# OpenMatchmaking/microservice-matchmaking

Measured on AMD Instinct MI355X. Metric: matched players/sec over 1M-player pool, higher is better.
Workload: dtype int32

## Files before the change

microservice_matchmaking_amd/csrc/mm_engine.hip:

```cpp
#include <hip/hip_runtime.h>

#include <stdint.h>
#include <stdio.h>
#include <stdlib.h>
#include <string.h>
#include <time.h>

#include <dlfcn.h>

#include <algorithm>
#include <mutex>
#include <cmath>
#include <new>
#include <vector>

#include "../../include/mm_engine.h"
#include "../../include/mm_wait.h"
#include <mm_gfx950.h>


#define MM_NO_SLOT 0xFFFFFFFFu
#define MM_ST_FREE 0
#define MM_ST_LIVE 1
#define MM_ST_CANCELLED 2
// ... 841 lines not shown
    hipStream_t stream;
    hipEvent_t ev[4];
    hipEvent_t ev_nx[2];
    bool ev_nx_set;
    hipEvent_t ev_grp[MM_MAX_GROUPS];
    int last_hip;
    int32_t* d_q_rating;
    uint32_t* d_q_cons;
    uint32_t* d_q_slot;
    ChainDev* d_chains;
    uint8_t* d_state;
    uint32_t* d_released;
    uint32_t* d_counters;
    uint32_t* d_wave_hist;
    size_t wave_hist_rows;
    int32_t* d_in_rating;
    uint32_t* d_in_cons;
    uint8_t* d_in_group;
    uint32_t* d_in_slot;
    uint32_t* d_in_sel;
    size_t in_cap;
    uint32_t* d_in_stamp;
    size_t in_stamp_cap;
    uint32_t* d_out_slots;
    float* d_out_score;
    uint32_t* d_out_pass;
    uint32_t out_slot_stride, out_rec_stride;
    PairChain* d_pchains;
    uint32_t* d_pk_key[2];
    uint32_t* d_pk_oidx[2];
    uint16_t* d_pk_nx16[2];
    uint32_t* d_pk_bits[2];
    uint32_t* d_pk_scratch;
    uint16_t* d_pk_wpre;
    uint16_t* d_pk_g16;
    uint32_t* d_pk_rec1;
    uint16_t* d_pk_exa[2];
    uint32_t* d_pk_bitsp[2];
    uint32_t* d_pk_headp[2];
    bool kp_rounds_off;
    uint32_t pair_pcool;
    uint32_t pair_pstops;
    unsigned long long* d_pk_pbar;
    uint32_t round_ctr;
    uint32_t* d_pk_tilectl;
    uint32_t* d_pack;
    uint4* d_pk_grec;
    uint32_t pk_gstride;
    PairChain* h_pchains;
    uint32_t* h_look_seq;
    uint32_t look_seq;
    uint32_t ps_hand[4][MM_MAX_GROUPS];
    mm_path_stats ps;
    mm_tuning tn;
    uint32_t pk_bits_stride, pk_max_tiles, pk_stride;
    unsigned long long live_upper;
    TeamChain* d_tchains;
    TeamChain* h_tchains;
    uint32_t* d_tk_chunk;
    uint32_t* d_tk_fv2;
    uint32_t* d_tk_fpos;
    uint16_t* d_tk_memb;
    uint32_t* d_tk_bitsB;
    uint32_t* d_tk_chunkB;
    uint32_t* d_tk_fdone;
    uint32_t team_seq;
    uint32_t* d_tk_sqi;
// ... 445 lines not shown
    MMTRY(dev_alloc(e, e->d_q_rating, e->n_chains * cap * sizeof(int32_t)));
    MMTRY(dev_alloc(e, e->d_q_cons, e->n_chains * cap * sizeof(uint32_t)));
    MMTRY(dev_alloc(e, e->d_q_slot, e->n_chains * cap * sizeof(uint32_t)));
    MMTRY(dev_alloc(e, e->d_chains, e->n_chains * sizeof(ChainDev)));
    MMTRY(dev_alloc(e, e->d_state, cap));
    MMTRY(dev_alloc(e, e->d_released, (cap + 64) * sizeof(uint32_t)));
    MMTRY(dev_alloc(e, e->d_pack, (size_t)MM_PACK_MAX * (MM_MAX_LOBBY + 2u) * sizeof(uint32_t)));
    MMTRY(dev_alloc(e, e->d_counters, 2 * sizeof(uint32_t)));
    e->out_slot_stride = (uint32_t)(cap + 64);
    e->out_rec_stride = (uint32_t)(cap / 2 + 16);
    MMTRY(dev_alloc(e, e->d_out_slots, (size_t)cfg->n_groups * e->out_slot_stride * sizeof(uint32_t)));
    MMTRY(dev_alloc(e, e->d_out_score, (size_t)cfg->n_groups * e->out_rec_stride * sizeof(float)));
    MMTRY(dev_alloc(e, e->d_out_pass, (size_t)cfg->n_groups * e->out_rec_stride * sizeof(uint32_t)));
    {
        e->pk_stride = (uint32_t)((cap + 63) & ~(size_t)63);
        const size_t gc = (size_t)cfg->n_groups * e->pk_stride;
        e->pk_bits_stride = (uint32_t)(cap / 32 + 4);
        MMTRY(dev_alloc(e, e->d_pchains, cfg->n_groups * sizeof(PairChain)));
        e->pk_max_tiles = (uint32_t)(cap / (PK_TMAX / 4u) + 2);
        for (int b = 0; b < 2; ++b) {
            MMTRY(dev_alloc(e, e->d_pk_key[b], (gc + 64) * sizeof(uint32_t)));
            MMTRY(dev_alloc(e, e->d_pk_oidx[b], gc * sizeof(uint32_t)));
            MMTRY(dev_alloc(e, e->d_pk_nx16[b], (gc + 64) * sizeof(uint16_t)));
            MMTRY(dev_alloc(e, e->d_pk_bits[b], (size_t)cfg->n_groups * e->pk_bits_stride * sizeof(uint32_t)));
        }
        MMTRY(dev_alloc(e, e->d_pk_scratch, gc * sizeof(uint32_t)));
        MMTRY(dev_alloc(e, e->d_pk_g16, (gc + 64) * sizeof(uint16_t)));
        MMTRY(dev_alloc(e, e->d_pk_rec1, gc * sizeof(uint32_t)));
        for (int b = 0; b < 2; ++b) {
            MMTRY(dev_alloc(e, e->d_pk_exa[b], (gc + 64) * sizeof(uint16_t)));
            MMTRY(dev_alloc(e, e->d_pk_bitsp[b], (size_t)cfg->n_groups * e->pk_bits_stride * sizeof(uint32_t)));
            MMTRY(dev_alloc(e, e->d_pk_headp[b], (size_t)cfg->n_groups * e->pk_max_tiles * sizeof(uint32_t)));
        }
        MMTRY(dev_alloc(e, e->d_pk_wpre, (size_t)cfg->n_groups * e->pk_bits_stride * sizeof(uint16_t)));
        MMTRY(dev_alloc(e, e->d_pk_tilectl, (size_t)TC_N * cfg->n_groups * e->pk_max_tiles * sizeof(uint32_t)));
        MMTRY(dev_alloc(e, e->d_pk_pbar, (size_t)MM_MAX_GROUPS * 2u * sizeof(unsigned long long) + 64u));
        e->pk_gstride = (uint32_t)(2u * (e->pk_stride / PK_GS) + 4u * PK_TMAX);
        MMTRY(dev_alloc(e, e->d_pk_grec, (size_t)cfg->n_groups * e->pk_gstride * sizeof(uint4)));
        HIPCHK(e, hipMemsetAsync(e->d_pk_grec, 0xFF, (size_t)cfg->n_groups * e->pk_gstride * sizeof(uint4), e->stream));
        MMTRY(pin_alloc(e, e->h_pchains, cfg->n_groups * sizeof(PairChain)));
        MMTRY(pin_alloc(e, e->h_rslots, (cap + (size_t)3 * MM_MAX_LOBBY * cfg->n_groups + 64) * sizeof(uint32_t)));
        MMTRY(pin_alloc(e, e->h_rscore, (cap / 2 + (size_t)3 * MM_MAX_LOBBY * cfg->n_groups + 64) * sizeof(float)));
        MMTRY(pin_alloc(e, e->h_rpass, (cap / 2 + (size_t)3 * MM_MAX_LOBBY * cfg->n_groups + 64) * sizeof(uint32_t)));
        HIPCHK(e, hipMemsetAsync(e->d_pchains, 0, cfg->n_groups * sizeof(PairChain), e->stream));
        e->tk_chunk_stride = (uint32_t)(e->pk_stride / TT_CH + 2);
        MMTRY(dev_alloc(e, e->d_tchains, cfg->n_groups * sizeof(TeamChain)));
        MMTRY(dev_alloc(e, e->d_tk_chunk, (size_t)cfg->n_groups * MM_MAX_ROLES * e->tk_chunk_stride * sizeof(uint32_t)));
        MMTRY(dev_alloc(e, e->d_tk_fv2, gc * sizeof(uint32_t)));
        e->tk_memb = 0;
        for (uint32_t k = 0; k < cfg->n_modes; ++k) {
            const uint32_t L = cfg->modes[k].teams * cfg->modes[k].team_size;
            if (L > 2u && L - 1u > e->tk_memb) e->tk_memb = L - 1u;
        }
        if (e->tk_memb) {
            MMTRY(dev_alloc(e, e->d_tk_fpos, gc * sizeof(uint32_t)));
            MMTRY(dev_alloc(e, e->d_tk_memb, gc * e->tk_memb * sizeof(uint16_t)));
            MMTRY(dev_alloc(e, e->d_tk_bitsB, (size_t)cfg->n_groups * e->pk_bits_stride * sizeof(uint32_t)));
            MMTRY(dev_alloc(e, e->d_tk_chunkB, (size_t)cfg->n_groups * MM_MAX_ROLES * e->tk_chunk_stride * sizeof(uint32_t)));
            MMTRY(dev_alloc(e, e->d_tk_sqi, gc * sizeof(uint32_t)));
            MMTRY(dev_alloc(e, e->d_tk_fdone, (size_t)cfg->n_groups * e->tk_chunk_stride * sizeof(uint32_t)));
            HIPCHK(e, hipMemsetAsync(e->d_tk_fdone, 0, (size_t)cfg->n_groups * e->tk_chunk_stride * sizeof(uint32_t), e->stream));
        }
        MMTRY(pin_alloc(e, e->h_tchains, cfg->n_groups * sizeof(TeamChain)));
        HIPCHK(e, hipMemsetAsync(e->d_tchains, 0, cfg->n_groups * sizeof(TeamChain), e->stream));
    }
    MMTRY(pin_alloc(e, e->h_chains, e->n_chains * sizeof(ChainDev)));
    MMTRY(pin_alloc(e, e->h_look_seq, 64));
// ... 485 lines not shown
    P.out_rec_stride = e->out_rec_stride;
    P.chains = e->d_chains;
    P.q_rating = e->d_q_rating;
    P.q_cons = e->d_q_cons;
    P.q_slot = e->d_q_slot;
    P.state = e->d_state;
    P.released = e->d_released;
    P.n_released = e->d_counters;
    P.out_slots = e->d_out_slots;
    P.out_score = e->d_out_score;
    P.out_pass = e->d_out_pass;
}

static int pair_walk(mm_engine* e, uint32_t mode, const ModeDev& M, bool purge)
{
    const mm_config& cfg = e->cfg;
    const uint32_t G = cfg.n_groups;
    PairParams P;
    walk_params_common(P, e, mode, purge);
    P.tune = e->tn.pair_tune;
    P.pinject = e->tn.pair_pinject;
    P.ptimeout0 = e->tn.pair_ptimeout_us * 100u;
    P.ptimeout1 = P.ptimeout0 * 40u;
    P.window = M.window > 0xFFFFFu ? 0xFFFFFu : M.window;
    P.eqmask = M.eqmask;
    P.bits_stride = e->pk_bits_stride;
    P.pstride = e->pk_stride;
    P.pchains = e->d_pchains;
    for (int b = 0; b < 2; ++b) {
        P.key[b] = e->d_pk_key[b]; P.oidx[b] = e->d_pk_oidx[b];
        P.nx16[b] = e->d_pk_nx16[b]; P.bits[b] = e->d_pk_bits[b];
    }
    P.scratch = e->d_pk_scratch;
    P.wpre = e->d_pk_wpre;
    P.g16 = e->d_pk_g16;
    P.rec2[0] = e->d_pk_scratch;
    P.rec2[1] = e->d_pk_rec1;
    for (int b = 0; b < 2; ++b) { P.exa[b] = e->d_pk_exa[b]; P.bitsp[b] = e->d_pk_bitsp[b]; P.headp[b] = e->d_pk_headp[b]; }
    P.tilectl = e->d_pk_tilectl;
    P.max_tiles = e->pk_max_tiles;
    P.grec = e->d_pk_grec;
    P.gstride = e->pk_gstride;
    P.grp = 0;
    P.pbar = e->d_pk_pbar;
    P.pxmask = (uint32_t*)(e->d_pk_pbar + MM_MAX_GROUPS);
    P.pyield = (uint32_t*)(e->d_pk_pbar + MM_MAX_GROUPS) + MM_MAX_GROUPS;
    const unsigned long long bound64 = e->live_upper < cfg.capacity ? e->live_upper : cfg.capacity;
    const uint32_t bound = (uint32_t)bound64;
    if (e->tn.pair_tune & 0x10000u) HIPCHK(e, hipMemsetAsync(e->d_pk_grec, 0, (size_t)G * e->pk_gstride * sizeof(uint4), e->stream));
    hipLaunchKernelGGL(kp_init, dim3(G), dim3(1024), 0, e->stream, P, cfg.capacity);
    hipLaunchKernelGGL(kp_pack, dim3((bound + 32u + 1023u) / 1024u, G), dim3(1024), 0, e->stream, P);
    {
        uint32_t seg = 256u, stage = NXI_STAGE;
        while (seg < NXI_SEG && (unsigned long long)bound > 8192ull * seg) seg <<= 1;
        if (e->tn.pair_nxseg) seg = e->tn.pair_nxseg;
        if (e->tn.pair_nxstage) stage = e->tn.pair_nxstage;
        if (stage < seg + 64u) stage = seg + 64u;
        if (stage > NXI_STAGE) stage = NXI_STAGE;
        const bool timing = (cfg.flags & MM_CFG_TIMING) != 0;
        if (timing) HIPCHK(e, hipEventRecord(e->ev_nx[0], e->stream));
        hipLaunchKernelGGL(kp_nx_init, dim3((bound + seg - 1u) / seg + 1u, G), dim3(NXI_THREADS), 0, e->stream, P, seg, stage);
        if (timing) { HIPCHK(e, hipEventRecord(e->ev_nx[1], e->stream)); e->ev_nx_set = true; }
    }
    HIPCHK(e, hipGetLastError());
    uint32_t tail_no[MM_MAX_GROUPS];
    bool tail_send = false;
    memset(e->ps_hand, 0, sizeof(e->ps_hand));
    if (bound >= PL_MAX) {
        uint32_t tiles = (bound + PK_T - 1u) / PK_T + 1u;
        if (tiles > e->pk_max_tiles) tiles = e->pk_max_tiles;
        bool after_persist = false;
        uint32_t last_tp = 0;
        uint32_t idle_looks = 0;
        unsigned long long last_progress = ~0ull;
        for (uint32_t guard = 0;; ++guard) {
            if (idle_looks > 64u) return MM_ERR_INTERNAL;
            MMTRY(look_launch(e, e->d_pchains, e->h_pchains, G * sizeof(PairChain)));
            MMTRY(look_wait(e));
            ++e->ps.host_looks;
            if (e->tn.debug && guard >= 200u && guard % 200u == 0u) {
                fprintf(stderr, "[mm-pair] look %u: cool-down %u, persist %d, last tile length %u;", guard, e->pair_pcool, (int)kp_rounds_on(e), last_tp);
                for (uint32_t g = 0; g < G; ++g) {
                    const PairChain& pc = e->h_pchains[g];
                    if (pc.fast) fprintf(stderr, " g%u[stage %u m %u qlen %u passes %u compact %u pfail 0x%x]", g, pc.stage, pc.m, pc.qlen, pc.passes, pc.want_compact, pc.pfail);
                }
                fprintf(stderr, "\n");
            }
            {
                unsigned long long progress = 0;
                for (uint32_t g = 0; g < G; ++g) {
                    const PairChain& pc = e->h_pchains[g];
                    if (pc.fast) progress += (unsigned long long)pc.passes + ((unsigned long long)pc.m << 32) + (pc.stage == PS_TILED ? 1u : 0u) + pc.want_compact;
                }
                idle_looks = progress == last_progress ? idle_looks + 1u : 0u;
                last_progress = progress;
            }
            bool tiled = false, compact = false;
            uint32_t longest = 0;
            for (uint32_t g = 0; g < G; ++g) {
                const PairChain& pc = e->h_pchains[g];
                P.bm[g] = 0;
                P.bbuf[g] = 0;
                if (!pc.fast || pc.stage != PS_TILED) continue;
                if (after_persist && pc.pfail && (pc.pfail & 0xFFu) == PF_YIELD) ++e->ps.pair_yields;
                if (after_persist && pc.pfail && (pc.pfail & 0xFFu) != PF_YIELD) {
                    ++e->pair_pstops;
                    e->pair_pcool = 16u;
                    const uint32_t why = pc.pfail & 0xFFu;
                    if (why == PF_XCD) { e->kp_rounds_off = true; ++e->ps.pair_stops_xcd; }
                    else if (why == PF_INJECT) ++e->ps.pair_stops_inject;
                    else ++e->ps.pair_stops_timeout;
                    e->ps.degraded = 1;
// ... 43 lines not shown
                    if (pc.qlen <= capq && pc.m > capq && capq >= PL_MAX) {
                        hipLaunchKernelGGL(kp_ask_compact, dim3(G), dim3(64), 0, e->stream, P, 1u << gl);
                        compact = true;
                    } else {
                        if (pc.m > e->tn.pair_ptiles * PK_TMAX) want_fit = true;
                        yield_q = capq;
                        yield_g = gl;
                    }
                }
            }
            uint32_t tp = PK_TMAX;
            bool persist = kp_rounds_on(e) && !compact && (longest + PK_TMAX - 1u) / PK_TMAX <= e->tn.pair_ptiles;
            if (persist && e->pair_pcool) { --e->pair_pcool; persist = false; e->ps.degraded = 1; }
            if (!kp_rounds_on(e) && !compact && (longest + PK_TMAX - 1u) / PK_TMAX <= e->tn.pair_ptiles) e->ps.degraded = 1;
            const uint32_t cap_p = e->tn.pair_ptiles < e->tn.pair_tiles_max ? e->tn.pair_ptiles : e->tn.pair_tiles_max;
            const uint32_t tiles_max = kp_rounds_on(e) ? cap_p : e->tn.pair_tiles_max;
            if (!e->tn.pair_tile_fixed)
                for (uint32_t cand = PK_TMAX / 4u; cand < PK_TMAX; cand <<= 1)
                    if ((longest + cand - 1u) / cand <= tiles_max) { tp = cand; break; }
            if (last_tp && tp > last_tp && !compact) {
                hipLaunchKernelGGL(kp_ask_compact, dim3(G), dim3(64), 0, e->stream, P, 0xFFFFFFFFu);
                compact = true;
                last_tp = 0;
            }
            tiles = (longest + tp - 1u) / tp;
#define TILE_LAUNCH(KERNEL, GRID, BLOCK, ...)                                                                              \
    do {                                                                                                                   \
        if (tp == PK_TMAX) hipLaunchKernelGGL(KERNEL<PK_TMAX>, GRID, BLOCK, 0, e->stream, __VA_ARGS__);                    \
        else if (tp == PK_TMAX / 2u) hipLaunchKernelGGL(KERNEL<PK_TMAX / 2u>, GRID, BLOCK, 0, e->stream, __VA_ARGS__);     \
        else hipLaunchKernelGGL(KERNEL<PK_TMAX / 4u>, GRID, BLOCK, 0, e->stream, __VA_ARGS__);                             \
    } while (0)
#define COMPACT_LAUNCH()                                                                                                   \
    do {                                                                                                                   \
        TILE_LAUNCH(kc_words, dim3(tiles, G), dim3(256), P);                                                               \
        TILE_LAUNCH(kc_plan, dim3(G), dim3(1024), P);                                                                      \
        TILE_LAUNCH(kc_scatter, dim3(tiles, G), dim3(1024), P);                                                            \
        TILE_LAUNCH(kc_commit, dim3(G), dim3(1024), P);                                                                    \
    } while (0)
            if (compact) {
                COMPACT_LAUNCH();
                HIPCHK(e, hipGetLastError());
                continue;
            }
            last_tp = tp;
            for (uint32_t g = 0; g < G; ++g) P.pyq[g] = 0;
            P.pyq[yield_g] = yield_q;
            {
                P.grp = (e->tn.pair_group_min && tiles >= e->tn.pair_group_min && tp == PK_TMAX) ? PK_GS : 0u;
                const uint32_t ngr = P.grp ? (tiles + P.grp - 1u) / P.grp : 0u;
                dim3 rgrid(tiles, G);
                P.xslots = 0;
                uint32_t tof[MM_MAX_GROUPS];
                for (uint32_t g = 0; g < G; ++g) tof[g] = P.bm[g] ? (P.bm[g] + tp - 1u) / tp : 0u;
                if (persist) {
                    const uint32_t slots = pair_xcd_map(P, tof, G, true);
                    if (slots) {
                        P.grp = 0;
                        const uint32_t K = e->tn.pair_pbatch, slice = MM_PERSIST_SLICE ? MM_PERSIST_SLICE : K + 1u;
                        for (uint32_t it = 0; it <= K; it += slice)
                            TILE_LAUNCH(kp_rounds, dim3(8u * slots), dim3(PT_THREADS), P, it, it + slice < K + 1u ? it + slice : K + 1u, K);
                        ++e->ps.pair_rounds_launches;
                        after_persist = true;
                        COMPACT_LAUNCH();
                        HIPCHK(e, hipGetLastError());
                        MMTRY(results_absorb(e, M.L));
                        MMTRY(results_send(e, sent_no, M.L, e->tn.results_early ? MM_RESULTS_MIN_PAIR : 0xFFFFFFFFu));
                        continue;
                    }
                    P.xslots = 0;
                }
                if (e->tn.pair_xcd) {
                    const uint32_t slots = pair_xcd_map(P, tof, G);
                    if (slots) rgrid = dim3(8u * slots);
                }
                uint32_t r = e->round_ctr;
                TILE_LAUNCH(kp_round, rgrid, dim3(PT_THREADS), P, r, 1u);
                ++r;
                if (P.grp) TILE_LAUNCH(kp_group, dim3(ngr, G), dim3(1024), P, r);
                for (uint32_t b = 0; b < (want_fit && e->tn.pair_batch > 12u ? 12u : e->tn.pair_batch); ++b) {
                    TILE_LAUNCH(kp_round, rgrid, dim3(PT_THREADS), P, r, 0u);
                    ++e->ps.pair_round_launches;
                    ++r;
                    if (P.grp) TILE_LAUNCH(kp_group, dim3(ngr, G), dim3(1024), P, r);
                }
                TILE_LAUNCH(kp_round_commit, dim3(tiles, G), dim3(256), P, r);
                hipLaunchKernelGGL(kp_round_stage, dim3(G), dim3(64), 0, e->stream, P, r);
                COMPACT_LAUNCH();
                e->round_ctr = r;
            }
#undef COMPACT_LAUNCH
#undef TILE_LAUNCH
            HIPCHK(e, hipGetLastError());
            MMTRY(results_absorb(e, M.L));
            MMTRY(results_send(e, sent_no, M.L, e->tn.results_early ? MM_RESULTS_MIN_PAIR : 0xFFFFFFFFu));
        }
    }
    hipLaunchKernelGGL(kp_late, dim3(G), dim3(PL_THREADS), 0, e->stream, P);
    hipLaunchKernelGGL(kp_finish, dim3(G), dim3(1024), 0, e->stream, P);
    HIPCHK(e, hipGetLastError());
    if (tail_send) {
        MMTRY(results_absorb(e, M.L));
        MMTRY(results_send(e, tail_no, M.L, e->tn.results_early ? MM_RESULTS_MIN_PAIR : 0xFFFFFFFFu));
    }
    return MM_OK;
}

static void report_team(const mm_engine* e)
{
    const uint32_t G = e->cfg.n_groups;
    for (uint32_t g = 0; g < G; ++g) {
        const TeamChain& t = e->h_tchains[g];
        const uint32_t np = t.passes + 1u;
        fprintf(stderr, "[mm-team] g%u fast %u m %u passes %u out %u left %u | cancel tick: head sat out %u, seated %u, lobby filtered %u, anchor moved %u x | "
                "kt_f, the middle chunk, cycles per pass: first loads %u, probes + lists %u, replacements %u, look-ups from scratch %u, barrier %u, step C %u; anchors at work per pass %u | "
                "F values written %u, changed after the first pass %u | kt_chase: sub-queue entries looked at by the stored lobby's fills %u, by %u look-ups %u\n",
                g, t.fast, t.m, t.passes, t.n_out, t.qlen,
                t.dbg[6] & 1u, (t.dbg[6] >> 1) & 1u, (t.dbg[6] >> 2) & 1u, t.dbg[7],
                t.tmk[0] / np, t.tmk[1] / np, t.tmk[2] / np, t.tmk[3] / np, t.tmk[4] / np, t.tmk[5] / np, t.dbg[2] / np, t.dbg[5], t.dbg[4],
                t.dbg[0], t.dbg[3], t.dbg[1]);
        if (t.lt[11])
            fprintf(stderr, "[mm-team] g%u kt_fc's chaser: %u passes, %u lobbies by F; cycles per pass: all %u, the chase loop %u, its hops by F %u, of them on kt_f's flags %u; "
                    "cycles per hop without the flags %u; %u look-ups, cycles each: starts %u, the roles' stretches %u, the members' records %u, seats + kills (the one a pass ends on) %u "
                    "(with MM_TEAM_LATE=0: kt_late keeps its own timers in the same words)\n",
                    g, t.lt[11], t.lt[12], 16u * (t.lt[9] / t.lt[11]), 16u * (t.lt[10] / t.lt[11]), 16u * (t.lt[13] / t.lt[11]), 16u * (t.lt[8] / t.lt[11]),
                    t.lt[12] ? (uint32_t)(16ull * (t.lt[13] - t.lt[8]) / t.lt[12]) : 0u,
                    t.lt[3], t.lt[3] ? 16u * (t.lt[4] / t.lt[3]) : 0u, t.lt[3] ? 16u * (t.lt[5] / t.lt[3]) : 0u, t.lt[3] ? 16u * (t.lt[6] / t.lt[3]) : 0u,
                    16u * (t.lt[7] / t.lt[11]));
    }
}

static void report_team_late(const mm_engine* e, const uint32_t* p0)
{
    const uint32_t G = e->cfg.n_groups;
    for (uint32_t g = 0; g < G; ++g) {
        const TeamChain& t = e->h_tchains[g];
// ... 1341 lines not shown
```

microservice_matchmaking_amd/csrc/mm_pair.inc:

```

#define PK_NO 0xFFFFFFFFu
#define PK_ABORT 0xFFFFFFFEu

#define NX_INV 0u
#define NX_NONE 0xFFFFu
#define NX_FAR 0xFFFEu

#ifndef PK_T
#define PK_T 8192u
#endif
enum : uint32_t { PK_TMAX = PK_T };
#undef PK_T
static constexpr uint32_t PK_T = PK_TMAX;
#ifndef PK_TILES_MAX
#define PK_TILES_MAX 40u
#endif
#define PK_XSEG 4u
#ifndef PK_GS
#define PK_GS 8u
#endif
#ifndef PK_GROUP_MIN
#define PK_GROUP_MIN 64u
#endif
#ifndef PL_MAX
#define PL_MAX 16384u
#endif
#define PL_THREADS 1024
#define PL_WORDS (PL_MAX / 32u)
#ifndef PL_COMPACT_MIN
#define PL_COMPACT_MIN 2048u
#endif
#define LNX_NONE 0xFFFFu
#define LNX_INV 0xFFFEu
#define PS_TILED 0u
#define PS_LATE 1u
#define PS_DONE 2u
#define TC_ENT 0u
#define TC_OFF 1u
#define TC_DISP 2u
#define TC_ALIVE 3u
#define TC_BASE 4u
#define TC_N 5u
#define DISP_NONE 0xFFFFFFFFu
#define DISP_SEATED 0xFFFFFFFEu
#define REC_CLEAN 0u
#define REC_PARTNER 1u
#define REC_FAR 2u
#define REC_NONE 3u
#define EV_NONE 0u
#define EV_DONE 1u
#define EV_COMPACT 2u

struct RoundState {
    uint32_t live;
    uint32_t done;
    uint32_t want_compact, rounds;
    uint32_t qlen, passes, n_out, has_anchor;
    uint32_t a_key, a_slot, a_cons, a_team;
    int32_t  a_rating;
    uint32_t pos0;
    uint32_t changed0, extra0;
    uint32_t a_oi;
    unsigned long long pairs, scanned;
};

struct PairChain {
    uint32_t fast;
    uint32_t m;
    uint32_t qlen;
    uint32_t buf;
    int32_t  rmin;
    uint32_t has_anchor;
    uint32_t a_key, a_slot, a_cons, a_team;
    int32_t  a_rating;
    uint32_t passes, n_out, before, err;
// ... 27 lines not shown
    uint32_t pstride;
    uint32_t tune;
    uint32_t purge;
    uint8_t* state;
    uint32_t* released;
    uint32_t* n_released;
    ChainDev* chains;
    PairChain* pchains;
    int32_t* q_rating;
    uint32_t* q_cons;
    uint32_t* q_slot;
    uint32_t* key[2];
    uint32_t* oidx[2];
    uint16_t* nx16[2];
    uint32_t* bits[2];
    uint32_t* scratch;
    uint16_t* g16;
    uint32_t* rec2[2];
    uint16_t* exa[2];
    uint32_t* bitsp[2];
    uint32_t* headp[2];
    uint4* grec;
    uint32_t grp;
    uint32_t xslots;
    uint32_t xseg[8][PK_XSEG];
    uint16_t xcnt[8][PK_XSEG];
    uint32_t gstride;
    unsigned long long* pbar;
    uint32_t* pxmask;
    uint32_t ptimeout0, ptimeout1;
    uint32_t pinject;
    uint32_t* pyield;
    uint32_t pyq[MM_MAX_GROUPS];
    uint16_t* wpre;
    uint32_t* tilectl;
    uint32_t max_tiles;
    uint32_t* out_slots;
    float* out_score;
    uint32_t* out_pass;
    uint32_t bm[MM_MAX_GROUPS];
    uint8_t bbuf[MM_MAX_GROUPS];
};

#define PK_DEAD 0x80000000u
#define PK_SPAN_BITS 19
#define PK_RMASK 0x7FFFFu
static __device__ __forceinline__ uint32_t pk_pack(int32_t r, uint32_t cons, int32_t rmin, uint32_t eqmask)
{
    return ((uint32_t)r - (uint32_t)rmin) | (((cons & eqmask) >> 4) << PK_SPAN_BITS);
}
static __device__ __forceinline__ uint32_t pk_rating(uint32_t k) { return k & PK_RMASK; }
static __device__ __forceinline__ void pk_bounds(uint32_t ka, uint32_t w, uint32_t& lo, uint32_t& rng)
{
    const uint32_t ra = ka & PK_RMASK, top = ka & ~PK_RMASK;
    const uint32_t rl = ra > w ? ra - w : 0u;
    const uint32_t rh = ra + w < PK_RMASK ? ra + w : PK_RMASK;
    lo = top | rl;
    rng = rh - rl;
}
static __device__ __forceinline__ bool pk_in(uint32_t kc, uint32_t lo, uint32_t rng) { return kc - lo <= rng; }
static __device__ __forceinline__ bool pk_fit(uint32_t ka, uint32_t kc, uint32_t w)
{
    uint32_t lo, rng;
    pk_bounds(ka, w, lo, rng);
    return pk_in(kc, lo, rng);
}

// ... 78 lines not shown
        pc->changed0 = changed0;
        pc->extra0 = extra0;
        pc->buf = 0;
        pc->rmin = lo;
        pc->has_anchor = has;
        pc->a_key = has ? pk_pack(a_rating, a_cons, lo, P.eqmask) : 0u;
        pc->a_slot = a_slot;
        pc->a_cons = a_cons;
        pc->a_team = team;
        pc->a_rating = a_rating;
        pc->passes = 0;
        pc->n_out = 0;
        pc->before = m + lb.n + (P.purge ? ch->purged : 0u);
        pc->err = 0;
        pc->pairs = 0;
        pc->scanned = 0;
        pc->tested = 0;
        pc->tested_nx = 0;
        for (int k = 0; k < 8; ++k) pc->dbg[k] = 0;
        pc->stage = m < PL_MAX ? PS_LATE : PS_TILED;
        pc->ntiles = (m + PK_T - 1u) / PK_T;
        pc->want_compact = 0;
        pc->cur_pass = 0;
        pc->new_m = m;
        pc->rounds = 0;
        pc->ghops = 0; pc->gtry = 0; pc->gstale = 0;
        for (int k = 0; k < 16; ++k) { pc->tm[k] = 0; pc->ptm[k] = 0; }
        pc->pfail = 0; pc->ppass = 0;
        for (int k = 0; k < 4; ++k) pc->pslow[k] = 0;
        pc->pxm = 0;
        P.pbar[g] = 0ull; P.pxmask[g] = 0u;
        if (g == 0u) *P.pyield = 0u;
    }
    if (m <= max_len) {
        const uint32_t nt = (m + PK_T - 1u) / PK_T;
        for (uint32_t t = tid; t < P.max_tiles; t += 1024) {
            P.tilectl[((size_t)TC_ENT * P.n_groups + g) * P.max_tiles + t] = PK_NO;
            P.tilectl[((size_t)TC_ALIVE * P.n_groups + g) * P.max_tiles + t] =
                t < nt ? dev_min_u32(PK_T, m - t * PK_T) : 0u;
        }
    }
}

__global__ __launch_bounds__(1024) void kp_pack(PairParams P)
{
    const uint32_t g = blockIdx.y;
    const PairChain* const pc = P.pchains + g;
    if (!pc->fast) return;
    const uint32_t m = pc->m;
    const uint32_t i = blockIdx.x * 1024u + threadIdx.x;
    const uint32_t c = P.mode * P.n_groups + g;
    const size_t qo = (size_t)c * P.capacity, po = (size_t)g * P.pstride;
    if (i < m) {
        P.key[0][po + i] = pk_pack(P.q_rating[qo + i], P.q_cons[qo + i], pc->rmin, P.eqmask);
        P.oidx[0][po + i] = i;
        P.nx16[0][po + i] = (uint16_t)NX_INV;
    }
    if ((i & 31u) == 0u && i < m + 32u) {
        const uint32_t left = i < m ? m - i : 0u;
        uint32_t wbits = left >= 32u ? 0xFFFFFFFFu : ((1u << left) - 1u);
        if (i == 0u && pc->extra0) wbits &= ~1u;
        P.bits[0][(size_t)g * P.bits_stride + (i >> 5)] = wbits;
    }
}

#define NXI_THREADS 512
#define NXI_SEG 2048u
#define NXI_STAGE 8192u
__global__ __launch_bounds__(NXI_THREADS) void kp_nx_init(PairParams P, uint32_t seg, uint32_t stage)
{
    __shared__ uint32_t s_k[NXI_STAGE];
    const uint32_t g = blockIdx.y;
    const PairChain* const pc = P.pchains + g;
    if (!pc->fast) return;
// ... 2127 lines not shown
    const uint32_t nw = (dev_min_u32(PK_T, m - t * PK_T) + 31u) >> 5;
    const uint32_t* const src = P.bitsp[cpar] + (size_t)g * P.bits_stride + w0;
    uint32_t* const dst = P.bits[pc->buf] + (size_t)g * P.bits_stride + w0;
    for (uint32_t i = tid; i < nw; i += 256) dst[i] = src[i];
    __syncthreads();
    if (t == 0 && tid == 0) {
        const RoundState S = pc->rs[cpar];
        pc->qlen = S.qlen; pc->passes = S.passes; pc->n_out = S.n_out; pc->has_anchor = S.has_anchor;
        pc->a_key = S.a_key; pc->a_slot = S.a_slot; pc->a_cons = S.a_cons; pc->a_team = S.a_team;
        pc->a_rating = S.a_rating; pc->pairs = S.pairs; pc->scanned = S.scanned; pc->rounds = S.rounds;
        pc->want_compact = S.want_compact;
        pc->pos0 = S.pos0; pc->changed0 = S.changed0; pc->extra0 = S.extra0;
    }
}

__global__ __launch_bounds__(64) void kp_ask_compact(PairParams P, uint32_t mask)
{
    const uint32_t g = blockIdx.x;
    PairChain* const pc = P.pchains + g;
    if (threadIdx.x == 0 && ((mask >> g) & 1u) && pc->fast && pc->stage == PS_TILED) pc->want_compact = 1u;
}

__global__ __launch_bounds__(64) void kp_round_stage(PairParams P, uint32_t r_next)
{
    const uint32_t g = blockIdx.x;
    PairChain* const pc = P.pchains + g;
    if (!pc->fast || pc->stage != PS_TILED) return;
    if (threadIdx.x == 0) {
        if (pc->rs[r_next & 1u].done) pc->stage = PS_DONE;
        else if (P.pyq[g] && pc->qlen <= P.pyq[g]) pc->want_compact = 1u;
    }
}

template <uint32_t TP>
__global__ __launch_bounds__(256) void kc_words(PairParams P)
{
    constexpr uint32_t PK_T = TP;
    (void)PK_T;
    __shared__ uint32_t s_wtot[4];
    const uint32_t g = blockIdx.y, t = blockIdx.x;
    const PairChain* const pc = P.pchains + g;
    if (!pc->fast || pc->stage != PS_TILED || !pc->want_compact || t >= (pc->m + PK_T - 1u) / PK_T) return;
    const int tid = threadIdx.x, lane = tid & 63, wave = tid >> 6;
    const uint32_t m = pc->m;
    const uint32_t w0 = t * (PK_T / 32u);
    const uint32_t nw = (dev_min_u32(PK_T, m - t * PK_T) + 31u) >> 5;
    const uint32_t* const bits = P.bits[pc->buf] + (size_t)g * P.bits_stride + w0;
    const uint32_t pcw = (uint32_t)tid < nw ? (uint32_t)__popc(bits[tid]) : 0u;
    const uint32_t incl = wave_incl_scan(pcw, lane);
    if (lane == 63) s_wtot[wave] = incl;
    __syncthreads();
    uint32_t offw = 0;
    for (int x = 0; x < wave; ++x) offw += s_wtot[x];
    if ((uint32_t)tid < nw) P.wpre[(size_t)g * P.bits_stride + w0 + tid] = (uint16_t)(offw + incl - pcw);
    if (tid == 255) tc_row(P, TC_ALIVE, g)[t] = offw + incl;
}

template <uint32_t TP>
__global__ __launch_bounds__(1024) void kc_plan(PairParams P)
{
    constexpr uint32_t PK_T = TP;
    (void)PK_T;
    const uint32_t g = blockIdx.x;
    PairChain* const pc = P.pchains + g;
    if (!pc->fast || pc->stage != PS_TILED || !pc->want_compact) return;
    __shared__ uint32_t s_total;
    const int tid = threadIdx.x;
    uint32_t* const talive = tc_row(P, TC_ALIVE, g);
    uint32_t* const tbase = tc_row(P, TC_BASE, g);
    if (tid == 0) {
        uint32_t run = 0;
        for (uint32_t t = 0; t < (pc->m + PK_T - 1u) / PK_T; ++t) { tbase[t] = run; run += talive[t]; }
        s_total = run;
        pc->new_m = run;
        if (run != pc->qlen) pc->err |= MM_ERRF_SEAT_INVARIANT;
    }
    __syncthreads();
    const uint32_t nm = s_total;
    uint32_t* const nbits = P.bits[pc->buf ^ 1u] + (size_t)g * P.bits_stride;
    for (uint32_t i = tid; i < (nm >> 5) + 2u; i += 1024) {
        const uint32_t lo = i << 5;
        nbits[i] = lo + 32u <= nm ? 0xFFFFFFFFu : (lo < nm ? (1u << (nm - lo)) - 1u : 0u);
    }
}

template <uint32_t TP>
__global__ __launch_bounds__(1024) void kc_scatter(PairParams P)
{
    constexpr uint32_t PK_T = TP;
    (void)PK_T;
    const uint32_t g = blockIdx.y, t = blockIdx.x;
    const PairChain* const pc = P.pchains + g;
    if (!pc->fast || pc->stage != PS_TILED || !pc->want_compact || t >= (pc->m + PK_T - 1u) / PK_T) return;
    const int tid = threadIdx.x;
    const uint32_t m = pc->m, buf = pc->buf;
    const size_t po = (size_t)g * P.pstride;
    const uint32_t* const bits = P.bits[buf] + (size_t)g * P.bits_stride;
    const uint16_t* const wpre = P.wpre + (size_t)g * P.bits_stride;
    const uint32_t* const tbase = tc_row(P, TC_BASE, g);
    const uint32_t base = t * PK_T;
    const uint32_t tl = dev_min_u32(PK_T, m - base);
    for (uint32_t x = tid; x < tl; x += 1024) {
        const uint32_t i = base + x;
        const uint32_t bw = bits[i >> 5];
        if (!((bw >> (i & 31u)) & 1u)) continue;
        const uint32_t r = tbase[t] + wpre[i >> 5] + (uint32_t)__popc(bw & ((1u << (i & 31u)) - 1u));
        P.key[buf ^ 1u][po + r] = P.key[buf][po + i];
        P.oidx[buf ^ 1u][po + r] = P.oidx[buf][po + i];
        const uint32_t o = P.nx16[buf][po + i];
        uint32_t no = NX_INV;
        if (o == NX_NONE) no = NX_NONE;
        else if (o != NX_INV && o != NX_FAR) {
            const uint32_t q = i + o;
            const uint32_t qw = q < m ? bits[q >> 5] : 0u;
            if ((qw >> (q & 31u)) & 1u) {
                const uint32_t rq = tbase[q / PK_T] + wpre[q >> 5] + (uint32_t)__popc(qw & ((1u << (q & 31u)) - 1u));
                no = rq - r;
            }
        }
        P.nx16[buf ^ 1u][po + r] = (uint16_t)no;
    }
}

template <uint32_t TP>
__global__ __launch_bounds__(1024) void kc_commit(PairParams P)
{
    constexpr uint32_t PK_T = TP;
    (void)PK_T;
    const uint32_t g = blockIdx.x;
    PairChain* const pc = P.pchains + g;
    if (threadIdx.x == 0) { P.pbar[g] = 0ull; P.pxmask[g] = 0u; if (g == 0u) *P.pyield = 0u; }
    if (!pc->fast || pc->stage != PS_TILED || !pc->want_compact) return;
    const int tid = threadIdx.x;
    const uint32_t nm = pc->new_m;
    const uint32_t nt = (nm + PK_T - 1u) / PK_T;
    uint32_t* const talive = tc_row(P, TC_ALIVE, g);
    for (uint32_t t = tid; t < P.max_tiles; t += 1024) talive[t] = t < nt ? dev_min_u32(PK_T, nm - t * PK_T) : 0u;
    __syncthreads();
    if (tid == 0) {
        pc->m = nm;
        pc->ntiles = nt;
        pc->buf ^= 1u;
        pc->want_compact = 0;
        if (nm < PL_MAX) pc->stage = PS_LATE;
    }
}

__global__ __launch_bounds__(1024) void kp_finish(PairParams P)
{
    __shared__ uint32_t wtot[16];
    const int tid = threadIdx.x, lane = tid & 63, wave = tid >> 6;
    const uint32_t g = blockIdx.x;
    PairChain* const pc = P.pchains + g;
    if (!pc->fast) return;
    const uint32_t c = P.mode * P.n_groups + g;
    ChainDev* const ch = P.chains + c;
    const size_t qo = (size_t)c * P.capacity, po = (size_t)g * P.pstride;
    const uint32_t m = pc->m;
    const uint32_t* const oidx = P.oidx[pc->buf] + po;
    const uint32_t* const bits = P.bits[pc->buf] + (size_t)g * P.bits_stride;
    uint32_t* const t_rating = P.key[pc->buf ^ 1u] + po;
    uint32_t* const t_cons = P.oidx[pc->buf ^ 1u] + po;
    uint32_t* const t_slot = P.scratch + po;
    uint32_t wr = 0;
    for (uint32_t base = 0; base < m; base += 1024u) {
        const uint32_t i = base + (uint32_t)tid;
        const bool live = i < m && ((bits[i >> 5] >> (i & 31u)) & 1u);
        const unsigned long long bm = __ballot(live);
        if (lane == 0) wtot[wave] = (uint32_t)__popcll(bm);
        __syncthreads();
        uint32_t off = wr, tot = 0;
        for (int x = 0; x < 16; ++x) {
            if (x < wave) off += wtot[x];
            tot += wtot[x];
        }
// ... 38 lines not shown
```

Baseline: 108.4 million.

## Fold compaction prefix sums into scatter and issue first chain look early

The compaction path drops the separate word-prefix and per-tile planning kernels. Each scatter block now recomputes its global offset by popcounting all bitmap words before its tile, then scans a small staged window of words in shared memory. The commit kernel recounts the survivors itself and rewrites the new bitmap, which removes the wpre buffer and the alive/base tile-control rows. The host also issues the first device-to-host chain look right after packing, overlapping it with the nx-init kernel. The cost is redundant prefix popcount work that grows with tile index, possible serial popcount loops for far neighbours, and some debug timing prints.

```diff
diff --git a/microservice_matchmaking_amd/csrc/mm_engine.hip b/microservice_matchmaking_amd/csrc/mm_engine.hip
--- a/microservice_matchmaking_amd/csrc/mm_engine.hip
+++ b/microservice_matchmaking_amd/csrc/mm_engine.hip
@@ -897,7 +897,6 @@
     uint16_t* d_pk_nx16[2];
     uint32_t* d_pk_bits[2];
     uint32_t* d_pk_scratch;
-    uint16_t* d_pk_wpre;
     uint16_t* d_pk_g16;
     uint32_t* d_pk_rec1;
     uint16_t* d_pk_exa[2];
@@ -1409,7 +1408,6 @@
             MMTRY(dev_alloc(e, e->d_pk_bitsp[b], (size_t)cfg->n_groups * e->pk_bits_stride * sizeof(uint32_t)));
             MMTRY(dev_alloc(e, e->d_pk_headp[b], (size_t)cfg->n_groups * e->pk_max_tiles * sizeof(uint32_t)));
         }
-        MMTRY(dev_alloc(e, e->d_pk_wpre, (size_t)cfg->n_groups * e->pk_bits_stride * sizeof(uint16_t)));
         MMTRY(dev_alloc(e, e->d_pk_tilectl, (size_t)TC_N * cfg->n_groups * e->pk_max_tiles * sizeof(uint32_t)));
         MMTRY(dev_alloc(e, e->d_pk_pbar, (size_t)MM_MAX_GROUPS * 2u * sizeof(unsigned long long) + 64u));
         e->pk_gstride = (uint32_t)(2u * (e->pk_stride / PK_GS) + 4u * PK_TMAX);
@@ -1961,7 +1959,6 @@
         P.nx16[b] = e->d_pk_nx16[b]; P.bits[b] = e->d_pk_bits[b];
     }
     P.scratch = e->d_pk_scratch;
-    P.wpre = e->d_pk_wpre;
     P.g16 = e->d_pk_g16;
     P.rec2[0] = e->d_pk_scratch;
     P.rec2[1] = e->d_pk_rec1;
@@ -1979,6 +1976,11 @@
     if (e->tn.pair_tune & 0x10000u) HIPCHK(e, hipMemsetAsync(e->d_pk_grec, 0, (size_t)G * e->pk_gstride * sizeof(uint4), e->stream));
     hipLaunchKernelGGL(kp_init, dim3(G), dim3(1024), 0, e->stream, P, cfg.capacity);
     hipLaunchKernelGGL(kp_pack, dim3((bound + 32u + 1023u) / 1024u, G), dim3(1024), 0, e->stream, P);
+    const bool look_early = bound >= PL_MAX && !e->tn.look_poll;
+    if (look_early) {
+        MMTRY(look_launch(e, e->d_pchains, e->h_pchains, G * sizeof(PairChain)));
+        HIPCHK(e, hipEventRecord(e->ev[3], e->stream));
+    }
     {
         uint32_t seg = 256u, stage = NXI_STAGE;
         while (seg < NXI_SEG && (unsigned long long)bound > 8192ull * seg) seg <<= 1;
@@ -2004,9 +2006,13 @@
         unsigned long long last_progress = ~0ull;
         for (uint32_t guard = 0;; ++guard) {
             if (idle_looks > 64u) return MM_ERR_INTERNAL;
-            MMTRY(look_launch(e, e->d_pchains, e->h_pchains, G * sizeof(PairChain)));
-            MMTRY(look_wait(e));
+            if (guard == 0u && look_early) HIPCHK(e, hipEventSynchronize(e->ev[3]));
+            else {
+                MMTRY(look_launch(e, e->d_pchains, e->h_pchains, G * sizeof(PairChain)));
+                MMTRY(look_wait(e));
+            }
             ++e->ps.host_looks;
+            const double t_look = e->tn.debug ? host_now_ms() : 0.0;
             if (e->tn.debug && guard >= 200u && guard % 200u == 0u) {
                 fprintf(stderr, "[mm-pair] look %u: cool-down %u, persist %d, last tile length %u;", guard, e->pair_pcool, (int)kp_rounds_on(e), last_tp);
                 for (uint32_t g = 0; g < G; ++g) {
@@ -2116,8 +2122,6 @@
     } while (0)
 #define COMPACT_LAUNCH()                                                                                                   \
     do {                                                                                                                   \
-        TILE_LAUNCH(kc_words, dim3(tiles, G), dim3(256), P);                                                               \
-        TILE_LAUNCH(kc_plan, dim3(G), dim3(1024), P);                                                                      \
         TILE_LAUNCH(kc_scatter, dim3(tiles, G), dim3(1024), P);                                                            \
         TILE_LAUNCH(kc_commit, dim3(G), dim3(1024), P);                                                                    \
     } while (0)
@@ -2147,8 +2151,11 @@
                         after_persist = true;
                         COMPACT_LAUNCH();
                         HIPCHK(e, hipGetLastError());
+                        const double t_enq = e->tn.debug ? host_now_ms() : 0.0;
                         MMTRY(results_absorb(e, M.L));
                         MMTRY(results_send(e, sent_no, M.L, e->tn.results_early ? MM_RESULTS_MIN_PAIR : 0xFFFFFFFFu));
+                        if (e->tn.debug) fprintf(stderr, "[mm-pair] look %u (kp_rounds): batch enqueued %.1f us after the look returned, match list sent %.1f us after that%s\n",
+                                                 guard, (t_enq - t_look) * 1e3, (host_now_ms() - t_enq) * 1e3, e->ev_copy_pending ? " (a send in flight)" : "");
                         continue;
                     }
                     P.xslots = 0;
@@ -2175,8 +2182,11 @@
 #undef COMPACT_LAUNCH
 #undef TILE_LAUNCH
             HIPCHK(e, hipGetLastError());
+            const double t_enq = e->tn.debug ? host_now_ms() : 0.0;
             MMTRY(results_absorb(e, M.L));
             MMTRY(results_send(e, sent_no, M.L, e->tn.results_early ? MM_RESULTS_MIN_PAIR : 0xFFFFFFFFu));
+            if (e->tn.debug) fprintf(stderr, "[mm-pair] look %u: batch enqueued %.1f us after the look returned, match list sent %.1f us after that%s\n",
+                                     guard, (t_enq - t_look) * 1e3, (host_now_ms() - t_enq) * 1e3, e->ev_copy_pending ? " (a send in flight)" : "");
         }
     }
     hipLaunchKernelGGL(kp_late, dim3(G), dim3(PL_THREADS), 0, e->stream, P);
@@ -2185,6 +2195,7 @@
     if (tail_send) {
         MMTRY(results_absorb(e, M.L));
         MMTRY(results_send(e, tail_no, M.L, e->tn.results_early ? MM_RESULTS_MIN_PAIR : 0xFFFFFFFFu));
+        if (e->tn.debug) fprintf(stderr, "[mm-pair] look behind the last batch: kp_late enqueued%s\n", e->ev_copy_pending ? " (a send in flight)" : "");
     }
     return MM_OK;
 }
diff --git a/microservice_matchmaking_amd/csrc/mm_pair.inc b/microservice_matchmaking_amd/csrc/mm_pair.inc
--- a/microservice_matchmaking_amd/csrc/mm_pair.inc
+++ b/microservice_matchmaking_amd/csrc/mm_pair.inc
@@ -38,9 +38,7 @@
 #define TC_ENT 0u
 #define TC_OFF 1u
 #define TC_DISP 2u
-#define TC_ALIVE 3u
-#define TC_BASE 4u
-#define TC_N 5u
+#define TC_N 3u
 #define DISP_NONE 0xFFFFFFFFu
 #define DISP_SEATED 0xFFFFFFFEu
 #define REC_CLEAN 0u
@@ -134,7 +132,6 @@
     uint32_t pinject;
     uint32_t* pyield;
     uint32_t pyq[MM_MAX_GROUPS];
-    uint16_t* wpre;
     uint32_t* tilectl;
     uint32_t max_tiles;
     uint32_t* out_slots;
@@ -279,14 +276,8 @@
         P.pbar[g] = 0ull; P.pxmask[g] = 0u;
         if (g == 0u) *P.pyield = 0u;
     }
-    if (m <= max_len) {
-        const uint32_t nt = (m + PK_T - 1u) / PK_T;
-        for (uint32_t t = tid; t < P.max_tiles; t += 1024) {
-            P.tilectl[((size_t)TC_ENT * P.n_groups + g) * P.max_tiles + t] = PK_NO;
-            P.tilectl[((size_t)TC_ALIVE * P.n_groups + g) * P.max_tiles + t] =
-                t < nt ? dev_min_u32(PK_T, m - t * PK_T) : 0u;
-        }
-    }
+    if (m <= max_len)
+        for (uint32_t t = tid; t < P.max_tiles; t += 1024) P.tilectl[((size_t)TC_ENT * P.n_groups + g) * P.max_tiles + t] = PK_NO;
 }
 
 __global__ __launch_bounds__(1024) void kp_pack(PairParams P)
@@ -2480,79 +2471,59 @@
     }
 }
 
+#define KC_REACH 3u
+
+static __device__ __forceinline__ uint32_t kc_count(const uint32_t* __restrict__ bits, uint32_t from, uint32_t to, uint32_t* s_part)
+{
+    const int tid = threadIdx.x, lane = tid & 63, wave = tid >> 6;
+    uint32_t c = 0;
+    for (uint32_t i = from + (uint32_t)tid; i < to; i += 1024u) c += (uint32_t)__popc(bits[i]);
+    for (int d = 1; d < 64; d <<= 1) c += (uint32_t)__shfl((int)c, lane ^ d);
+    __syncthreads();
+    if (lane == 0) s_part[wave] = c;
+    __syncthreads();
+    uint32_t sum = 0;
+    for (int x = 0; x < 16; ++x) sum += s_part[x];
+    return sum;
+}
+
 template <uint32_t TP>
-__global__ __launch_bounds__(256) void kc_words(PairParams P)
+__global__ __launch_bounds__(1024) void kc_scatter(PairParams P)
 {
     constexpr uint32_t PK_T = TP;
-    (void)PK_T;
-    __shared__ uint32_t s_wtot[4];
+    constexpr uint32_t WT = PK_T / 32u;
+    static_assert(KC_REACH * WT <= 1024u, "a thread per staged bitmap word");
+    __shared__ uint32_t s_wp[KC_REACH * WT + 1u];
+    __shared__ uint32_t s_part[16];
     const uint32_t g = blockIdx.y, t = blockIdx.x;
     const PairChain* const pc = P.pchains + g;
     if (!pc->fast || pc->stage != PS_TILED || !pc->want_compact || t >= (pc->m + PK_T - 1u) / PK_T) return;
     const int tid = threadIdx.x, lane = tid & 63, wave = tid >> 6;
-    const uint32_t m = pc->m;
-    const uint32_t w0 = t * (PK_T / 32u);
-    const uint32_t nw = (dev_min_u32(PK_T, m - t * PK_T) + 31u) >> 5;
-    const uint32_t* const bits = P.bits[pc->buf] + (size_t)g * P.bits_stride + w0;
-    const uint32_t pcw = (uint32_t)tid < nw ? (uint32_t)__popc(bits[tid]) : 0u;
-    const uint32_t incl = wave_incl_scan(pcw, lane);
-    if (lane == 63) s_wtot[wave] = incl;
-    __syncthreads();
-    uint32_t offw = 0;
-    for (int x = 0; x < wave; ++x) offw += s_wtot[x];
-    if ((uint32_t)tid < nw) P.wpre[(size_t)g * P.bits_stride + w0 + tid] = (uint16_t)(offw + incl - pcw);
-    if (tid == 255) tc_row(P, TC_ALIVE, g)[t] = offw + incl;
-}
-
-template <uint32_t TP>
-__global__ __launch_bounds__(1024) void kc_plan(PairParams P)
-{
-    constexpr uint32_t PK_T = TP;
-    (void)PK_T;
-    const uint32_t g = blockIdx.x;
-    PairChain* const pc = P.pchains + g;
-    if (!pc->fast || pc->stage != PS_TILED || !pc->want_compact) return;
-    __shared__ uint32_t s_total;
-    const int tid = threadIdx.x;
-    uint32_t* const talive = tc_row(P, TC_ALIVE, g);
-    uint32_t* const tbase = tc_row(P, TC_BASE, g);
-    if (tid == 0) {
-        uint32_t run = 0;
-        for (uint32_t t = 0; t < (pc->m + PK_T - 1u) / PK_T; ++t) { tbase[t] = run; run += talive[t]; }
-        s_total = run;
-        pc->new_m = run;
-        if (run != pc->qlen) pc->err |= MM_ERRF_SEAT_INVARIANT;
-    }
-    __syncthreads();
-    const uint32_t nm = s_total;
-    uint32_t* const nbits = P.bits[pc->buf ^ 1u] + (size_t)g * P.bits_stride;
-    for (uint32_t i = tid; i < (nm >> 5) + 2u; i += 1024) {
-        const uint32_t lo = i << 5;
-        nbits[i] = lo + 32u <= nm ? 0xFFFFFFFFu : (lo < nm ? (1u << (nm - lo)) - 1u : 0u);
-    }
-}
-
-template <uint32_t TP>
-__global__ __launch_bounds__(1024) void kc_scatter(PairParams P)
-{
-    constexpr uint32_t PK_T = TP;
-    (void)PK_T;
-    const uint32_t g = blockIdx.y, t = blockIdx.x;
-    const PairChain* const pc = P.pchains + g;
-    if (!pc->fast || pc->stage != PS_TILED || !pc->want_compact || t >= (pc->m + PK_T - 1u) / PK_T) return;
-    const int tid = threadIdx.x;
     const uint32_t m = pc->m, buf = pc->buf;
     const size_t po = (size_t)g * P.pstride;
     const uint32_t* const bits = P.bits[buf] + (size_t)g * P.bits_stride;
-    const uint16_t* const wpre = P.wpre + (size_t)g * P.bits_stride;
-    const uint32_t* const tbase = tc_row(P, TC_BASE, g);
+    const uint32_t w0 = t * WT;
+    const uint32_t nwin = dev_min_u32(KC_REACH * WT, ((m + 31u) >> 5) - w0);
+    const uint32_t pre = kc_count(bits, 0u, w0, s_part);
+    {
+        const uint32_t pcw = (uint32_t)tid < nwin ? (uint32_t)__popc(bits[w0 + tid]) : 0u;
+        const uint32_t incl = wave_incl_scan(pcw, lane);
+        __syncthreads();
+        if (lane == 63) s_part[wave] = incl;
+        __syncthreads();
+        uint32_t offw = 0;
+        for (int x = 0; x < wave; ++x) offw += s_part[x];
+        if ((uint32_t)tid < nwin) s_wp[tid] = offw + incl - pcw;
+        if ((uint32_t)tid + 1u == nwin) s_wp[nwin] = offw + incl;
+        __syncthreads();
+    }
     const uint32_t base = t * PK_T;
     const uint32_t tl = dev_min_u32(PK_T, m - base);
     for (uint32_t x = tid; x < tl; x += 1024) {
         const uint32_t i = base + x;
         const uint32_t bw = bits[i >> 5];
         if (!((bw >> (i & 31u)) & 1u)) continue;
-        const uint32_t r = tbase[t] + wpre[i >> 5] + (uint32_t)__popc(bw & ((1u << (i & 31u)) - 1u));
+        const uint32_t r = pre + s_wp[(i >> 5) - w0] + (uint32_t)__popc(bw & ((1u << (i & 31u)) - 1u));
         P.key[buf ^ 1u][po + r] = P.key[buf][po + i];
         P.oidx[buf ^ 1u][po + r] = P.oidx[buf][po + i];
         const uint32_t o = P.nx16[buf][po + i];
@@ -2562,8 +2533,13 @@
             const uint32_t q = i + o;
             const uint32_t qw = q < m ? bits[q >> 5] : 0u;
             if ((qw >> (q & 31u)) & 1u) {
-                const uint32_t rq = tbase[q / PK_T] + wpre[q >> 5] + (uint32_t)__popc(qw & ((1u << (q & 31u)) - 1u));
-                no = rq - r;
+                uint32_t rq;
+                if ((q >> 5) - w0 < nwin) rq = pre + s_wp[(q >> 5) - w0];
+                else {
+                    rq = pre + s_wp[nwin];
+                    for (uint32_t wq = w0 + nwin; wq < (q >> 5); ++wq) rq += (uint32_t)__popc(bits[wq]);
+                }
+                no = rq + (uint32_t)__popc(qw & ((1u << (q & 31u)) - 1u)) - r;
             }
         }
         P.nx16[buf ^ 1u][po + r] = (uint16_t)no;
@@ -2575,20 +2551,26 @@
 {
     constexpr uint32_t PK_T = TP;
     (void)PK_T;
+    __shared__ uint32_t s_part[16];
     const uint32_t g = blockIdx.x;
     PairChain* const pc = P.pchains + g;
     if (threadIdx.x == 0) { P.pbar[g] = 0ull; P.pxmask[g] = 0u; if (g == 0u) *P.pyield = 0u; }
     if (!pc->fast || pc->stage != PS_TILED || !pc->want_compact) return;
     const int tid = threadIdx.x;
-    const uint32_t nm = pc->new_m;
-    const uint32_t nt = (nm + PK_T - 1u) / PK_T;
-    uint32_t* const talive = tc_row(P, TC_ALIVE, g);
-    for (uint32_t t = tid; t < P.max_tiles; t += 1024) talive[t] = t < nt ? dev_min_u32(PK_T, nm - t * PK_T) : 0u;
+    const uint32_t buf = pc->buf;
+    const uint32_t nm = kc_count(P.bits[buf] + (size_t)g * P.bits_stride, 0u, (pc->m + 31u) >> 5, s_part);
+    uint32_t* const nbits = P.bits[buf ^ 1u] + (size_t)g * P.bits_stride;
+    for (uint32_t i = tid; i < (nm >> 5) + 2u; i += 1024) {
+        const uint32_t lo = i << 5;
+        nbits[i] = lo + 32u <= nm ? 0xFFFFFFFFu : (lo < nm ? (1u << (nm - lo)) - 1u : 0u);
+    }
     __syncthreads();
     if (tid == 0) {
+        if (nm != pc->qlen) pc->err |= MM_ERRF_SEAT_INVARIANT;
+        pc->new_m = nm;
         pc->m = nm;
-        pc->ntiles = nt;
-        pc->buf ^= 1u;
+        pc->ntiles = (nm + PK_T - 1u) / PK_T;
+        pc->buf = buf ^ 1u;
         pc->want_compact = 0;
         if (nm < PL_MAX) pc->stage = PS_LATE;
     }
```

Measured after the change: 102.8 million. 5.2% lower.
